# takkasila/practical_path_guiding_lab

Measured on AMD Instinct MI355X. Metric: Msamples/s guided, veach-ajar 1920x1080 max_depth 13, higher is better.
Workload: dtype f32; 1 GPU; veach-ajar 1920x1080, max_depth 13, 16 one-sample training passes (main.py:192, 218) per step in one batched launch (the whole film), guided iteration 6 (SD-tree trained by rendering iterations 0-5, 252 spp); full PathGuidingIntegrator.sample(): camera rays, NEE, BSDF/SD-tree MIS, record list, po...; spp_per_pass=16, passes_per_launch=16, steps_per_launch=1, kd_leaves=21429, quad_records=1675769, jump_bits=6, kd_grid_bits=6, bytes_jump_tables=1404370944, pixels_per_rank_min=2073600, pixels_per_rank_max=2073600

## Files before the change

practical_path_guiding_lab_amd/csrc/pg_probe.hip:

```cpp
#include <string>
#include <type_traits>
#include <vector>

#include "pg_render_dev.hpp"
#include "pg_render_stages.hpp"
#include "pg_scene_state.hpp"

using namespace pg;

namespace {

constexpr uint64_t kProbeMaxRays = 1ull << 20;
static_assert(kProbeMaxRays * (uint64_t)kOvfStack <= 0xffffffffull, "pg_scene_intersect: the overflow strips are indexed by 32 bits");

struct ProbeArgs {
	Shapes shapes;
	uint64_t n;
	const float *o, *d, *tmax;
	float *t, *uv;
	int32_t *prim;
	uint2 *ovf;
};

template <int kLevel, bool kAny, int kForm>
__global__ __launch_bounds__(kRBlock) void k_probe_intersect(ProbeArgs p)
{
	constexpr int kStack = kForm == 1 ? kShadeStack : kLdsStack;
	constexpr int kTop = kForm == 1 ? kShadeTopNodes : kBvhTopNodes;
	__shared__ uint2 s_stack[kStack][kRBlock];
	const uint64_t tid = (uint64_t)blockIdx.x * kRBlock + threadIdx.x;
	BvhStack stk = bvh_stack(&s_stack[0][threadIdx.x], p.ovf, (uint32_t)tid * (uint32_t)kOvfStack, kStack);
	if (kForm != 2) {
		__shared__ u32x4_t s_top[kTop * kBvhNodeQuads];
		RenderArgs a;
		a.shapes = p.shapes;
		stage_bvh_top<kTop>(s_top, a, stk);
	}
	if (tid >= p.n) return;
	const v3 o = ld3(p.o + 3 * tid), d = ld3(p.d + 3 * tid);
	float t, bu = 0.0f, bv = 0.0f;
	const int prim = intersect<kLevel, kAny, kForm == 1>(p.shapes, o, d, p.tmax[tid], t, stk, bu, bv);
	p.t[tid] = t;
	p.prim[tid] = prim;
	p.uv[2 * tid] = bu;
	p.uv[2 * tid + 1] = bv;
}

template <int kLevel, bool kAny>
auto intersect_form(int form) -> void (*)(ProbeArgs)
{
	if (form == 0) return k_probe_intersect<kLevel, kAny, 0>;
	if (form == 1) return k_probe_intersect<kLevel, kAny, 1>;
	return k_probe_intersect<kLevel, kAny, 2>;
}
// ... 314 lines not shown
```

practical_path_guiding_lab_amd/csrc/pg_render_dev.hpp:

```cpp
#pragma once

#include "pg_context.hpp"
#include "pg_descent.hpp"
#include "pg_kernels.hpp"
#include "pg_scene_layout.hpp"

#define PG_OUTLINE __forceinline__

namespace pg {

constexpr int kRBlock = 256;
static_assert(kRBlock == kStageThreads, "stage_kd_planes copies one plane per thread");
constexpr float kInvPiF = 0.31830988618379067154f;
constexpr float kRayEps = 1e-4f;
constexpr float kShadowEps = 1e-3f;

struct v3 {
	float x, y, z;
};
__device__ __forceinline__ v3 V(float x, float y, float z) { v3 r = {x, y, z}; return r; }
__device__ __forceinline__ v3 vadd(v3 a, v3 b) { return V(a.x + b.x, a.y + b.y, a.z + b.z); }
__device__ __forceinline__ v3 vsub(v3 a, v3 b) { return V(a.x - b.x, a.y - b.y, a.z - b.z); }
__device__ __forceinline__ v3 vmul(v3 a, v3 b) { return V(a.x * b.x, a.y * b.y, a.z * b.z); }
__device__ __forceinline__ v3 vscale(v3 a, float s) { return V(a.x * s, a.y * s, a.z * s); }
// ... 62 lines not shown
typedef __attribute__((address_space(3))) uint32_t LdsWord;
typedef __attribute__((address_space(3))) u32x4_t LdsQuad;
struct BvhStack {
	LdsWord *lds;
	uint2 *ovf;
	uint32_t ovf_first;
	const LdsQuad *top;
	uint32_t n_top;
	int n_lds;
	__device__ __forceinline__ void push(int sp, uint32_t ref, float t) const
	{
		if (sp < n_lds) {
			lds[sp * (2 * kRBlock)] = ref;
			lds[sp * (2 * kRBlock) + 1] = __float_as_uint(t);
		} else ovf[ovf_first + (uint32_t)(sp - n_lds)] = make_uint2(ref, __float_as_uint(t));
	}
	__device__ __forceinline__ uint2 at(int sp) const
	{
		const volatile LdsWord *w = lds + (sp < n_lds ? sp : n_lds - 1) * (2 * kRBlock);
		uint2 e = make_uint2(w[0], w[1]);
		if (sp >= n_lds) e = ovf[ovf_first + (uint32_t)(sp - n_lds)];
		return e;
	}
	__device__ __forceinline__ void push_ref(int sp, uint32_t ref) const
	{
		if (sp < n_lds) lds[sp * (2 * kRBlock)] = ref;
		else ovf[ovf_first + (uint32_t)(sp - n_lds)].x = ref;
	}
	__device__ __forceinline__ uint32_t ref_at(int sp) const
	{
		const volatile LdsWord *w = lds + (sp < n_lds ? sp : n_lds - 1) * (2 * kRBlock);
		uint32_t r = w[0];
		if (sp >= n_lds) r = ovf[ovf_first + (uint32_t)(sp - n_lds)].x;
		return r;
	}
};
__device__ __forceinline__ BvhStack bvh_stack(uint2 *lds_column, uint2 *ovf, uint32_t ovf_first, int n_lds = kLdsStack)
{
	BvhStack s;
	s.n_lds = n_lds;
	s.lds = (LdsWord *)lds_column;
	s.ovf = ovf;
	s.ovf_first = ovf_first;
	s.top = nullptr; s.n_top = 0;
	return s;
}

__device__ __forceinline__ v3 box_face_normal(const float *B, int face)
{
	const v3 n = ld3(B + BOX_NORMALS + 3 * (face >> 1));
	return (face & 1) ? V(-n.x, -n.y, -n.z) : n;
}

__device__ __forceinline__ bool bvh_box_hit(float lox, float loy, float loz, float hix, float hiy, float hiz, v3 o,
                                            v3 inv, bool negx, bool negy, bool negz, float bt, float &tmin_out)
{
	const float nx = ((negx ? hix : lox) - o.x) * inv.x, fx = ((negx ? lox : hix) - o.x) * inv.x;
	const float ny = ((negy ? hiy : loy) - o.y) * inv.y, fy = ((negy ? loy : hiy) - o.y) * inv.y;
	const float nz = ((negz ? hiz : loz) - o.z) * inv.z, fz = ((negz ? loz : hiz) - o.z) * inv.z;
	const float tmin = __builtin_fmaxf(__builtin_fmaxf(__builtin_fmaxf(nx, ny), nz), 0.0f);
	const float tmax = __builtin_fminf(__builtin_fminf(__builtin_fminf(fx, fy), fz), bt);
	tmin_out = tmin;
	return tmin <= tmax * 1.0000004f;
}

__device__ __forceinline__ bool bvh_box_hit_nf(float nxp, float nyp, float nzp, float fxp, float fyp, float fzp, v3 o, v3 inv,
                                               float bt, float &tmin_out)
// ... 93 lines not shown
	int best, sp, budget;
	uint32_t next;
};
__device__ __forceinline__ void bvh_rows(v3 d, int &nx, int &fx, int &ny, int &fy, int &nz, int &fz)
{
	const bool ngx = (__float_as_uint(d.x) >> 31) != 0u, ngy = (__float_as_uint(d.y) >> 31) != 0u, ngz = (__float_as_uint(d.z) >> 31) != 0u;
	constexpr int lo = BVH_BOXES * 4, hi = lo + BVH_HI_ROW * (int)kBvhRowBytes, row = (int)kBvhRowBytes;
	nx = ngx ? hi : lo; fx = ngx ? lo : hi;
	ny = ngy ? hi + row : lo + row; fy = ngy ? lo + row : hi + row;
	nz = ngz ? hi + 2 * row : lo + 2 * row; fz = ngz ? lo + 2 * row : hi + 2 * row;
}

__device__ __forceinline__ void bvh_begin(BvhWalk &w, const Shapes &sh, v3 o, v3 d, float bt, int best)
{
	w.o = o; w.d = d;
	w.inv = V(1.0f / d.x, 1.0f / d.y, 1.0f / d.z);
	bvh_rows(d, w.row_nx, w.row_fx, w.row_ny, w.row_fy, w.row_nz, w.row_fz);
	w.bt = bt; w.bu = 0.0f; w.bv = 0.0f;
	w.best = best; w.sp = 0;
	w.budget = 8 * sh.n_bvh_nodes + 8;
	w.next = 0;
}

template <bool kSlim = false, bool kAny = false>
__device__ __forceinline__ void bvh_node_step(BvhWalk &w, const Shapes &sh, const BvhStack &stk)
{
	const float kInf = __builtin_huge_valf();
	int row_nx = w.row_nx, row_fx = w.row_fx, row_ny = w.row_ny, row_fy = w.row_fy, row_nz = w.row_nz, row_fz = w.row_fz;
	if (kSlim) {
		v3 d = w.d;
		asm volatile("" : "+v"(d.x), "+v"(d.y), "+v"(d.z));
		bvh_rows(d, row_nx, row_fx, row_ny, row_fy, row_nz, row_fz);
	}
	const char *B = reinterpret_cast<const char *>(sh.bvh);
	const uint32_t nb = w.next * kBvhNodeBytes;
	uint4 nx4, ny4, nz4, fx4, fy4, fz4, rf;
	if (w.next < stk.n_top) {
		const LdsQuad *T = stk.top + w.next * (uint32_t)kBvhNodeQuads;
#define PG_Q(r) ({ const u32x4_t q_ = T[r]; make_uint4(q_.x, q_.y, q_.z, q_.w); })
		nx4 = PG_Q(row_nx >> 4); ny4 = PG_Q(row_ny >> 4); nz4 = PG_Q(row_nz >> 4);
		fx4 = PG_Q(row_fx >> 4); fy4 = PG_Q(row_fy >> 4); fz4 = PG_Q(row_fz >> 4); rf = PG_Q(BVH_REFS / BVH_WIDTH);
#undef PG_Q
	} else {
		nx4 = gather16(B + (nb + (uint32_t)row_nx)); ny4 = gather16(B + (nb + (uint32_t)row_ny)); nz4 = gather16(B + (nb + (uint32_t)row_nz));
		fx4 = gather16(B + (nb + (uint32_t)row_fx)); fy4 = gather16(B + (nb + (uint32_t)row_fy)); fz4 = gather16(B + (nb + (uint32_t)row_fz));
		rf = gather16(B + (nb + kBvhRefsByte));
	}
	uint32_t r0 = rf.x, r1 = rf.y, r2 = rf.z, r3 = rf.w;
	float t0, t1, t2, t3;
#define PG_F(v) __uint_as_float(v)
	const bool h0 = bvh_box_hit_nf(PG_F(nx4.x), PG_F(ny4.x), PG_F(nz4.x), PG_F(fx4.x), PG_F(fy4.x), PG_F(fz4.x), w.o, w.inv, w.bt, t0);
	const bool h1 = bvh_box_hit_nf(PG_F(nx4.y), PG_F(ny4.y), PG_F(nz4.y), PG_F(fx4.y), PG_F(fy4.y), PG_F(fz4.y), w.o, w.inv, w.bt, t1);
	const bool h2 = bvh_box_hit_nf(PG_F(nx4.z), PG_F(ny4.z), PG_F(nz4.z), PG_F(fx4.z), PG_F(fy4.z), PG_F(fz4.z), w.o, w.inv, w.bt, t2);
	const bool h3 = bvh_box_hit_nf(PG_F(nx4.w), PG_F(ny4.w), PG_F(nz4.w), PG_F(fx4.w), PG_F(fy4.w), PG_F(fz4.w), w.o, w.inv, w.bt, t3);
#undef PG_F
	if (!(r0 != kBvhNone && h0)) { r0 = kBvhNone; t0 = kInf; }
	if (!(r1 != kBvhNone && h1)) { r1 = kBvhNone; t1 = kInf; }
	if (!(r2 != kBvhNone && h2)) { r2 = kBvhNone; t2 = kInf; }
	if (!(r3 != kBvhNone && h3)) { r3 = kBvhNone; t3 = kInf; }
	if (kAny) {
		const bool n0 = r0 != kBvhNone, n1 = !n0 && r1 != kBvhNone, n2 = !n0 && !n1 && r2 != kBvhNone;
		w.next = n0 ? r0 : (n1 ? r1 : (n2 ? r2 : r3));
		if (n1) r1 = kBvhNone;
		if (n2) r2 = kBvhNone;
		if (!n0 && !n1 && !n2) r3 = kBvhNone;
		if (r3 != kBvhNone) { stk.push_ref(w.sp, r3); ++w.sp; }
		if (r2 != kBvhNone) { stk.push_ref(w.sp, r2); ++w.sp; }
		if (r1 != kBvhNone) { stk.push_ref(w.sp, r1); ++w.sp; }
		--w.budget;
		return;
	}
	bvh_cswap(t0, r0, t1, r1);
	bvh_cswap(t2, r2, t3, r3);
	bvh_cswap(t0, r0, t2, r2);
	bvh_cswap(t1, r1, t3, r3);
	bvh_cswap(t1, r1, t2, r2);
	if (r3 != kBvhNone) { stk.push(w.sp, r3, t3); ++w.sp; }
	if (r2 != kBvhNone) { stk.push(w.sp, r2, t2); ++w.sp; }
	if (r1 != kBvhNone) { stk.push(w.sp, r1, t1); ++w.sp; }
	w.next = r0;
	--w.budget;
}

__device__ __forceinline__ void bvh_tri_test(BvhWalk &w, v3 v0, v3 e1, v3 e2, int prim)
{
	const v3 o = w.o, d = w.d;
	const v3 p = V(d.y * e2.z - d.z * e2.y, d.z * e2.x - d.x * e2.z, d.x * e2.y - d.y * e2.x);
	const float det = dot3(e1, p);
	if (det == 0.0f) return;
	const float inv_det = 1.0f / det;
	const v3 s = vsub(o, v0);
	const float u = dot3(s, p) * inv_det;
	if (!(u >= 0.0f && u <= 1.0f)) return;
	const v3 q = V(s.y * e1.z - s.z * e1.y, s.z * e1.x - s.x * e1.z, s.x * e1.y - s.y * e1.x);
	const float v = dot3(d, q) * inv_det;
	if (!(v >= 0.0f && u + v <= 1.0f)) return;
	const float t = dot3(e2, q) * inv_det;
	if (t > 0.0f && t < w.bt) { w.bt = t; w.best = prim; w.bu = u; w.bv = v; }
}

__device__ __forceinline__ void bvh_leaf_step(BvhWalk &w, const Shapes &sh, int tri_base)
{
	const uint32_t first = bvh_leaf_first(w.next), count = bvh_leaf_count(w.next);
	for (uint32_t i = first; i < first + count; ++i) {
		const float *T = sh.tris + (size_t)i * kTriStride;
		v3 v0 = ld3(T + TRI_V0);
		const v3 e1 = ld3(T + TRI_E1), e2 = ld3(T + TRI_E2);
		asm volatile("" : "+v"(v0.x), "+v"(v0.y), "+v"(v0.z));
		bvh_tri_test(w, v0, e1, e2, tri_base + (int)i);
	}
}

template <bool kAny = false>
__device__ __forceinline__ void bvh_pop(BvhWalk &w, const BvhStack &stk)
{
	w.next = kBvhNone;
	if (kAny) {
		if (w.sp && w.budget > 0) {
			--w.sp;
			w.next = stk.ref_at(w.sp);
			--w.budget;
		}
		return;
	}
	while (w.sp && w.next == kBvhNone && w.budget > 0) {
		--w.sp;
		const uint2 e = stk.at(w.sp);
		if (__uint_as_float(e.y) <= w.bt * 1.0000004f) w.next = e.x;
		--w.budget;
	}
}

template <int kGeneral, bool kAny = false, bool kSlim = false>
__device__ __forceinline__ int intersect(const Shapes &sh, v3 o, v3 d, float tmax, float &t_out, const BvhStack &stk,
                                         float &bu, float &bv)
{
	int best = -1;
	float bt = tmax;
	intersect_linear<kGeneral>(sh, o, d, bt, best);
	if (kGeneral >= 2 && sh.n_bvh_nodes && !(kAny && best >= 0)) {
		const int tri_base = sh.first_tri();
		BvhWalk w;
		bvh_begin(w, sh, o, d, bt, best);
		while (true) {
			while (!(w.next & kBvhLeafBit) && w.budget > 0) {
				bvh_node_step<kSlim, kAny>(w, sh, stk);
				if (w.next == kBvhNone) bvh_pop<kAny>(w, stk);
			}
			if (w.next != kBvhNone && (w.next & kBvhLeafBit)) {
				bvh_leaf_step(w, sh, tri_base);
				if (kAny && w.best >= 0) break;
			}
			bvh_pop<kAny>(w, stk);
			if (w.next == kBvhNone) break;
		}
		bt = w.bt; best = w.best;
		if (w.best >= tri_base) { bu = w.bu; bv = w.bv; }
	}
	t_out = bt;
	return best;
}


template <int kGeneral, bool kAny = false>
__device__ __forceinline__ int intersect(const Shapes &sh, v3 o, v3 d, float tmax, float &t_out)
{
	static_assert(kGeneral < 2, "mesh scenes pass their BVH stack");
	const BvhStack none = bvh_stack(nullptr, nullptr, 0u);
	float bu, bv;
	return intersect<kGeneral, kAny>(sh, o, d, tmax, t_out, none, bu, bv);
}

__device__ __forceinline__ v3 texture_eval(const Shapes &sh, int index, float u, float v)
{
	const uint32_t *T = sh.textures + (size_t)index * kTextureStride;
	static_assert(TEX_KIND == 0 && TEX_WIDTH == 1 && TEX_HEIGHT == 2 && TEX_FIRST == 3 && TEX_COLOR0 == 4 && TEX_COLOR1 == 7 &&
	              TEX_UV_SCALE == 10 && TEX_UV_OFFSET == 12, "texture_eval names the words of the groups by .x .y .z .w");
	const uint4 t0 = *reinterpret_cast<const uint4 *>(T + TEX_KIND), t2 = *reinterpret_cast<const uint4 *>(T + TEX_COLOR1 + 1),
	            t3 = *reinterpret_cast<const uint4 *>(T + TEX_UV_OFFSET);
	const float uu = __uint_as_float(t2.z) * u + __uint_as_float(t3.x);
	const float vv = __uint_as_float(t2.w) * v + __uint_as_float(t3.y);
	if (t0.x == TEX_CHECKERBOARD) {
		const uint4 t1 = *reinterpret_cast<const uint4 *>(T + TEX_COLOR0);
		const float fu = uu - __builtin_floorf(uu), fv = vv - __builtin_floorf(vv);
		const bool mx = fu > 0.5f, my = fv > 0.5f;
		return mx == my ? V(__uint_as_float(t1.x), __uint_as_float(t1.y), __uint_as_float(t1.z))
		                : V(__uint_as_float(t1.w), __uint_as_float(t2.x), __uint_as_float(t2.y));
	}
	const int W = (int)t0.y, H = (int)t0.z;
	float x = uu * (float)W - 0.5f, y = vv * (float)H - 0.5f;
	if (!(fabs_(x) < 1e9f)) x = 0.0f;
	if (!(fabs_(y) < 1e9f)) y = 0.0f;
	const float fx = __builtin_floorf(x), fy = __builtin_floorf(y);
// ... 597 lines not shown
	uint32_t *prev_quad;
	uint8_t *hit0;
	uint64_t *rng_state, *rng_inc;
	uint32_t *ray_of;
	float *r_bsdf, *r_tb, *r_tr, *r_nee, *r_wp;
	uint2 *r_slot;
	uint32_t *r_tree;
	const uint4 *st_in;
	uint4 *st_out;
	const uint64_t *inc_in;
	uint64_t *inc_out;
	uint16_t *sort_key;
	const uint32_t *perm;
	uint32_t n_sort;
	uint4 *carry_in, *carry_out;
	uint4 *Lq;
	uint32_t *ws;
	uint2 *bvh_ovf;
	uint32_t *cast_count, *shadow_count, *shadow_list;
};


constexpr int kBvhTopNodes = 48;
template <int kNodes>
__device__ __forceinline__ void stage_bvh_top(u32x4_t *s_top, const RenderArgs &a, BvhStack &stk)
{
	const uint32_t n = a.shapes.n_bvh_nodes < kNodes ? (uint32_t)a.shapes.n_bvh_nodes : (uint32_t)kNodes;
	constexpr int kLoads = (kNodes * kBvhNodeQuads + kRBlock - 1) / kRBlock;
	if (n) {
		u32x4_t v[kLoads];
#pragma unroll
		for (int k = 0; k < kLoads; ++k) {
			const uint32_t i = threadIdx.x + (uint32_t)k * kRBlock;
			v[k] = reinterpret_cast<const u32x4_t *>(a.shapes.bvh)[i < n * (uint32_t)kBvhNodeQuads ? i : 0u];
		}
#pragma unroll
		for (int k = 0; k < kLoads; ++k) {
			const uint32_t i = threadIdx.x + (uint32_t)k * kRBlock;
			if (i < n * (uint32_t)kBvhNodeQuads) s_top[i] = v[k];
		}
	}
	__syncthreads();
	stk.top = (const LdsQuad *)s_top;
	stk.n_top = n;
}
constexpr int kShadeTopNodes = 40;
constexpr int kShadeStack = 6;
static_assert(kShadeStack >= kMinLdsStack && kShadeStack <= kLdsStack, "k_wave_shade: LDS stack depth");

constexpr uint32_t kTailPaths = 128u * 1024u;
__host__ __device__ constexpr bool tail_checkpoint(int bounce, int max_depth)
{
	return max_depth > 8 && bounce >= 4 && bounce + 1 < max_depth &&
	       (bounce < 8 || (bounce < 16 && bounce % 2 == 0) || bounce % 4 == 0);
}
typedef const __attribute__((address_space(4))) uint32_t *ConstU32Ptr;
__device__ __forceinline__ uint32_t live_final(const RenderArgs &a, int j)
{
	return reinterpret_cast<ConstU32Ptr>(reinterpret_cast<uintptr_t>(a.live_count))[j];
}
__device__ __forceinline__ uint64_t records_before(const RenderArgs &a)
{
	uint64_t r = a.n_lanes;
	for (int j = 0; j + 1 < a.bounce; ++j) r += live_final(a, j);
	return r;
}

__device__ __forceinline__ bool tail_took_over(const RenderArgs &a, int bounce)
{
	if (a.max_depth <= 8) return false;
	for (int c = 4; c <= bounce; ++c)
// ... 56 lines not shown
```

practical_path_guiding_lab_amd/csrc/pg_render_wave.hip:

```cpp
#include "pg_render_stages.hpp"

namespace pg {

enum : int {
	WS_HIT_PRIM = 0, WS_HIT_T, WS_HIT_U, WS_HIT_V,
	WS_P, WS_NG = WS_P + 3,
	WS_FLAGS = WS_NG + 3,
	WS_U, WS_LE = WS_U + 10,
	WS_DS_D = WS_LE + 3, WS_DS_PDF = WS_DS_D + 3, WS_EM_W, WS_BV_EM = WS_EM_W + 3, WS_BP_EM = WS_BV_EM + 3,
	WS_SH_O, WS_SH_D = WS_SH_O + 3, WS_SH_T = WS_SH_D + 3,
	WS_WO_T, WS_ETA = WS_WO_T + 3,
	WS_RNG_LO, WS_RNG_HI,
	WS_OCC,
	WS_PDF_NEE, WS_PDF_TREE,
	WS_FWD, WS_FWD_THR = WS_FWD, WS_FWD_L = WS_FWD_THR + 4, WS_FWD_INC = WS_FWD_L + 4,
	WS_COUNT = WS_FWD_INC + 2
};

__device__ __forceinline__ void store_geo_position(const RenderArgs &a, uint32_t *geo, uint64_t rec_slot, v3 p)
{
	const uint64_t S = a.n_lanes * (uint64_t)a.max_depth;
	float *gf = reinterpret_cast<float *>(geo);
	PG_ST(gf + (GEO_P + 0) * S + rec_slot, p.x); PG_ST(gf + (GEO_P + 1) * S + rec_slot, p.y); PG_ST(gf + (GEO_P + 2) * S + rec_slot, p.z);
}
// ... 107 lines not shown
		ray_d = st_v3(q1);
		if (want_cls && tid < (uint64_t)a.n_sort)
			cls_ahead = (int)lane_class_ahead(st_u64(q0.w, q1.w), st_u64(q5.x, q5.y), a.frac);
	}
	HitRec h;
	h.u = 0.0f; h.v = 0.0f;
	h.prim = intersect<kLevel, false>(a.shapes, ray_o, ray_d, __builtin_huge_valf(), h.t, stk, h.u, h.v);
	if (a.carry_in) {
		*st_rec(a.carry_in, tid, PS_HIT) = st_q_hit(h);
		if (tid < (uint64_t)a.n_sort) a.sort_key[tid] = (uint16_t)(h.prim >= 0 ? vertex_sort_key(a, vadd(ray_o, vscale(ray_d, h.t)), cls_ahead) : 0xfffeu);
		return;
	}
	wsputu(a, WS_HIT_PRIM, tid, (uint32_t)h.prim);
	wsput(a, WS_HIT_T, tid, h.t);
	wsput(a, WS_HIT_U, tid, h.u);
	wsput(a, WS_HIT_V, tid, h.v);
}

constexpr int kRefillIdle = 16;
constexpr uint32_t kCastChunk = 128;
template <int kLevel, bool kFirst>
__global__ __launch_bounds__(kRBlock) __attribute__((amdgpu_waves_per_eu(7))) void k_wave_cast(RenderArgs a)
{
	__shared__ uint2 s_stack[kLdsStack][kRBlock];
	if (!kFirst && tail_took_over(a, a.bounce)) return;
	const uint32_t total = kFirst ? (uint32_t)a.n_lanes : live_final(a, a.bounce - 1);
	const uint32_t gtid = blockIdx.x * kRBlock + threadIdx.x, n_static = gridDim.x * kRBlock;
	if (blockIdx.x * kRBlock >= total) return;
	const unsigned wl = threadIdx.x & 63u;
	const Shapes &sh = a.shapes;
	__shared__ u32x4_t s_top[kBvhTopNodes * kBvhNodeQuads];
	BvhStack stk = bvh_stack(&s_stack[0][threadIdx.x], a.bvh_ovf, gtid * (uint32_t)kOvfStack);
	stage_bvh_top<kBvhTopNodes>(s_top, a, stk);
	const int tri_base = sh.first_tri();
	BvhWalk w;
	w.next = kBvhNone; w.sp = 0; w.budget = 0; w.best = -1; w.bt = 0.0f; w.bu = 0.0f; w.bv = 0.0f;
	bool has = false, first_round = true;
	bool exhausted = n_static >= total;
	uint32_t pool_next = 0, pool_end = 0;
	const uint32_t n_waves = n_static / 64u;
	uint64_t chunk = gtid / 64u;
	uint32_t my = 0;
	for (;;) {
		const unsigned long long idle = __ballot(!has);
		const uint32_t n_idle = (uint32_t)__popcll(idle);
		if (first_round || (!exhausted && n_idle >= (uint32_t)kRefillIdle)) {
			uint32_t idx = 0xffffffffu;
			if (first_round) idx = gtid;
			else {
				if (pool_next == pool_end) {
					const uint64_t begin = (uint64_t)n_static + chunk * kCastChunk;
					chunk += n_waves;
					if (begin >= (uint64_t)total) exhausted = true;
					else {
						pool_next = (uint32_t)begin;
// ... 281 lines not shown
			if (a.perm) {
				q2 = ws4(a, WS_FWD_THR, tid);
				q4 = ws4(a, WS_FWD_L, tid);
			} else {
				q2 = st_load(a.st_in, a, PS_THR, tid);
				q4 = st_load(a.st_in, a, PS_L, tid);
			}
			thr = st_v3(q2);
			ior = st_ior(q2);
			L = st_v3(q4);
			lane = st_lane(q4);
		}
		cont = stage_b<kLevel>(a, rng, thr, L, ior, A, g, occluded, lane, rec_base + tid, (uint32_t)a.bounce, ray_o, ray_d,
		                       prev_pdf, delta);
		p_here = A.p;
		if (kFirst) a.hit0[lane] = (A.flags & F_VALID) ? 1 : 0;
		if (!cont) end_path(a, lane, L);
	}
	append_survivors<kRBlock>(a, cont, ray_o, ray_d, thr, ior, delta, p_here, prev_pdf, L, lane, rng, s_wave, s_base, s_oct, s_rec);
}

constexpr int kShadeStage = 128;
constexpr int kShadeStash = 12;
constexpr int kShadeWalkQuads = kShadeStack * kRBlock / 2 + kShadeTopNodes * kBvhNodeQuads + kShadeStash * kRBlock / 4;
constexpr int kShadeLdsQuads = kShadeStage * PS_ENTRIES > kShadeWalkQuads ? kShadeStage * PS_ENTRIES : kShadeWalkQuads;
static_assert(PS_SPARE * kRBlock <= kShadeLdsQuads, "k_wave_shade: the records' seven entries per thread must fit the dynamic LDS");
template <int kLevel, bool kFirst>
__device__ __forceinline__ void shade_body(const RenderArgs &a)
{
	__shared__ float s_planes[3 * kKdGridPlanes];
	__shared__ uint32_t s_wave[kRBlock / 64];
	__shared__ uint32_t s_base;
	__shared__ uint32_t s_oct[kRBlock / 64][8];
	extern __shared__ uint4 s_dyn[];
	uint64_t tid;
	bool alive;
	if (!wave_entry<kFirst>(a, tid, alive)) return;
#ifndef PG_SHADE_PHASES
#define PG_SHADE_PHASES 0
#endif
#if PG_SHADE_PHASES
	__shared__ unsigned long long s_ph[kRBlock / 64][10];
	if ((threadIdx.x & 63u) == (unsigned)__builtin_ctzll(__ballot(1))) {
		s_ph[threadIdx.x >> 6][8] = (unsigned long long)clock64();
		s_ph[threadIdx.x >> 6][7] = 0ull;
	}
#define PG_PHASE(i)                                                                                                          \
	if (a.ph && (threadIdx.x & 63u) == (unsigned)__builtin_ctzll(__ballot(1))) {                                            \
		const unsigned long long t_now = (unsigned long long)clock64();                                                      \
		unsigned long long *row = s_ph[threadIdx.x >> 6];                                                                    \
		row[i] = t_now - row[8];                                                                                             \
		row[8] = t_now;                                                                                                      \
		row[7] |= 1ull << (i);                                                                                               \
	}
#else
#define PG_PHASE(i)
#endif
	constexpr int kPlaneLoads = 1, kTopLoads = (kShadeTopNodes * kBvhNodeQuads + kRBlock - 1) / kRBlock;
	float pl_pre[kPlaneLoads];
	u32x4_t top_pre[kTopLoads];
#pragma unroll
	for (int k = 0; k < kPlaneLoads; ++k) pl_pre[k] = 0.0f;
#pragma unroll
	for (int k = 0; k < kTopLoads; ++k) top_pre[k] = u32x4_t{0u, 0u, 0u, 0u};
	const uint32_t n_top = a.shapes.n_bvh_nodes < kShadeTopNodes ? (uint32_t)a.shapes.n_bvh_nodes : (uint32_t)kShadeTopNodes;
#pragma unroll
	for (int k = 0; k < kPlaneLoads; ++k)
		if (a.tree.kd_grid != nullptr && threadIdx.x + k * kRBlock < 3u * kKdGridPlanes) pl_pre[k] = a.tree.kd_planes[threadIdx.x + k * kRBlock];
#pragma unroll
	for (int k = 0; k < kTopLoads; ++k)
		if (threadIdx.x + k * kRBlock < n_top * 8u) top_pre[k] = reinterpret_cast<const u32x4_t *>(a.shapes.bvh)[threadIdx.x + k * kRBlock];
	uint4 cq0 = make_uint4(0u, 0u, 0u, 0u), cq1 = cq0, cq2 = cq0, cq3 = cq0, cq4 = cq0, cq5 = cq0, cq6 = cq0;
	uint32_t coop_place = (uint32_t)tid;
	const bool coop = !kFirst && a.perm != nullptr;
	if (coop) {
		if (alive && tid < (uint64_t)a.n_sort) coop_place = a.perm[tid];
		if (!alive) coop_place = 0u;
		const uint32_t l = threadIdx.x & 63u, wbase = threadIdx.x & ~63u, q = l & 7u;
		uint4 g[8];
#pragma unroll
		for (uint32_t k = 0; k < 8u; ++k) {
			const uint32_t j = k * 8u + (l >> 3);
			const uint32_t pj = (uint32_t)__shfl((int)coop_place, (int)j, 64);
			g[k] = gather16(st_rec(a.carry_in, pj, (int)q));
		}
#pragma unroll
		for (uint32_t k = 0; k < 8u; ++k)
			if (q < (uint32_t)PS_SPARE) s_dyn[q * kRBlock + wbase + k * 8u + (l >> 3)] = g[k];
		__builtin_amdgcn_fence(__ATOMIC_RELEASE, "wavefront");
		__builtin_amdgcn_wave_barrier();
		__builtin_amdgcn_fence(__ATOMIC_ACQUIRE, "wavefront");
		cq0 = s_dyn[PS_RAY_O * kRBlock + threadIdx.x]; cq1 = s_dyn[PS_RAY_D * kRBlock + threadIdx.x]; cq2 = s_dyn[PS_THR * kRBlock + threadIdx.x];
		cq3 = s_dyn[PS_PREV * kRBlock + threadIdx.x]; cq4 = s_dyn[PS_L * kRBlock + threadIdx.x]; cq5 = s_dyn[PS_INC * kRBlock + threadIdx.x];
		cq6 = s_dyn[PS_HIT * kRBlock + threadIdx.x];
		__syncthreads();
	}
	uint2 *s_stack = reinterpret_cast<uint2 *>(s_dyn);
	u32x4_t *s_top = reinterpret_cast<u32x4_t *>(s_dyn) + kShadeStack * kRBlock / 2;
	BvhStack stk = bvh_stack(s_stack + threadIdx.x, a.bvh_ovf, (uint32_t)tid * (uint32_t)kOvfStack, kShadeStack);
#pragma unroll
	for (int k = 0; k < kPlaneLoads; ++k)
		if (a.tree.kd_grid != nullptr && threadIdx.x + k * kRBlock < 3u * kKdGridPlanes) s_planes[threadIdx.x + k * kRBlock] = pl_pre[k];
	if (a.tree.kd_grid != nullptr)
		for (uint32_t i = threadIdx.x + kPlaneLoads * kRBlock; i < 3u * kKdGridPlanes; i += kRBlock) s_planes[i] = a.tree.kd_planes[i];
#pragma unroll
	for (int k = 0; k < kTopLoads; ++k)
		if (threadIdx.x + k * kRBlock < n_top * 8u) s_top[threadIdx.x + k * kRBlock] = top_pre[k];
	__syncthreads();
	stk.top = (const LdsQuad *)s_top;
	stk.n_top = n_top;
	bool cont = false;
	v3 ray_o = V(0, 0, 0), ray_d = V(0, 0, 1), thr = V(1, 1, 1), L = V(0, 0, 0), p_here = V(0, 0, 0), prev_p = V(0, 0, 0);
	float ior = 1.0f, prev_pdf = 1.0f;
	bool delta = false, prev_delta = true;
	uint64_t lane = tid;
	Pcg32 rng;
	rng.state = 0; rng.inc = 1;
	uint64_t rec_base = 0;
	if (!kFirst) {
		rec_base = records_before(a);
		rec_base = (uint64_t)__builtin_amdgcn_readfirstlane((uint32_t)rec_base) |
		           ((uint64_t)__builtin_amdgcn_readfirstlane((uint32_t)(rec_base >> 32)) << 32);
	}
	if (alive) {
		HitRec h;
		const bool from_rec = !kFirst && a.perm != nullptr;
		uint32_t place = (uint32_t)tid;
		if (!coop && from_rec && tid < (uint64_t)a.n_sort) place = a.perm[tid];
		if (kFirst) {
			camera_ray(a, tid, rng, ray_o, ray_d);
			h.u = 0.0f; h.v = 0.0f;
			h.prim = intersect<kLevel, false, true>(a.shapes, ray_o, ray_d, __builtin_huge_valf(), h.t, stk, h.u, h.v);
		} else if (from_rec) {
// ... 9 lines not shown
			prev_delta = st_delta(q2);
			prev_p = st_v3(q3);
			prev_pdf = st_wf(q3);
			h = st_hit(q6);
		} else {
			const uint4 q0 = st_load(a.st_in, a, PS_RAY_O, tid), q1 = st_load(a.st_in, a, PS_RAY_D, tid);
			rng.state = st_u64(q0.w, q1.w);
			rng.inc = a.inc_in[tid];
			ray_o = st_v3(q0); ray_d = st_v3(q1);
			const uint4 q2 = st_load(a.st_in, a, PS_THR, tid), q3 = st_load(a.st_in, a, PS_PREV, tid);
			thr = st_v3(q2);
			{ const uint4 q4 = st_load(a.st_in, a, PS_L, tid); ior = st_ior(q2); L = st_v3(q4); lane = st_lane(q4); }
			prev_delta = st_delta(q2);
			prev_p = st_v3(q3);
			prev_pdf = st_wf(q3);
			h = ws_hit(a, tid);
		}
		StageA A;
		PG_PHASE(0)
		stage_a1<kLevel>(a, rng, ray_o, ray_d, thr, prev_p, prev_pdf, prev_delta, h, (uint32_t)a.bounce, A);
		asm volatile("" : "+v"(A.flags), "+v"(A.wi.x), "+v"(A.wi.y), "+v"(A.wi.z), "+v"(A.p.x), "+v"(A.p.y), "+v"(A.p.z),
		                  "+v"(A.ng.x), "+v"(A.ng.y), "+v"(A.ng.z), "+v"(A.refl.x), "+v"(A.refl.y), "+v"(A.refl.z));
		asm volatile("" : "+v"(A.ds_d.x), "+v"(A.ds_d.y), "+v"(A.ds_d.z), "+v"(A.ds_pdf), "+v"(A.bp_em), "+v"(A.n.x), "+v"(A.n.y), "+v"(A.n.z));
		float *stash = reinterpret_cast<float *>(s_dyn) + (kShadeStack * kRBlock * 2 + kShadeTopNodes * 32) + threadIdx.x;
		stash[0 * kRBlock] = A.Le.x; stash[1 * kRBlock] = A.Le.y; stash[2 * kRBlock] = A.Le.z;
		stash[3 * kRBlock] = A.bv_em.x; stash[4 * kRBlock] = A.bv_em.y; stash[5 * kRBlock] = A.bv_em.z;
		stash[6 * kRBlock] = A.em_w.x; stash[7 * kRBlock] = A.em_w.y; stash[8 * kRBlock] = A.em_w.z;
		stash[9 * kRBlock] = thr.x; stash[10 * kRBlock] = thr.y; stash[11 * kRBlock] = thr.z;
		bool occluded = false;
		PG_PHASE(1)
		if (a.dc) {
			const unsigned long long m = __ballot((A.flags & F_NEED_SHADOW) != 0u);
			if ((threadIdx.x & 63u) == (unsigned)__builtin_ctzll(__ballot(1))) {
				atomicAdd(&a.dc->body_waves, 1ull);
				if (m) { atomicAdd(&a.dc->shadow_waves, 1ull); atomicAdd(&a.dc->shadow_lanes, (unsigned long long)__popcll(m)); }
			}
		}
		if (A.flags & F_NEED_SHADOW) {
			float th, bu, bv;
			occluded = intersect<kLevel, true, true>(a.shapes, A.sh_o, A.sh_d, A.sh_tmax, th, stk, bu, bv) >= 0;
		}
		PG_PHASE(2)
		asm volatile("" : "+v"(A.n.x), "+v"(A.n.y), "+v"(A.n.z), "+v"(A.mat));
		stage_a2<kLevel>(a, rng, A);
		asm volatile("" : "+v"(A.wo.x), "+v"(A.wo.y), "+v"(A.wo.z), "+v"(A.bsdf_w.x), "+v"(A.bsdf_w.y), "+v"(A.bsdf_w.z),
		                  "+v"(A.bsdf_pdf), "+v"(A.flags));
		if (kLevel >= 3) asm volatile("" : "+v"(A.eta));
		GuideOut g = guide_none(A.wo);
		PG_PHASE(3)
		if (guide_has_work(a, A.flags)) stage_guide(a, s_planes, rng, A.p, A.ds_d, (A.flags & F_SMP_TREE) ? V(0, 0, 0) : A.wo, A.flags, g);
		if (a.record && (A.flags & F_VALID)) store_slots(a, rec_base + tid, g);
		PG_PHASE(4)
		asm volatile("" : "+v"(A.n.x), "+v"(A.n.y), "+v"(A.n.z), "+v"(A.mat));
		A.Le = V(stash[0 * kRBlock], stash[1 * kRBlock], stash[2 * kRBlock]);
		A.bv_em = V(stash[3 * kRBlock], stash[4 * kRBlock], stash[5 * kRBlock]);
		A.em_w = V(stash[6 * kRBlock], stash[7 * kRBlock], stash[8 * kRBlock]);
		thr = V(stash[9 * kRBlock], stash[10 * kRBlock], stash[11 * kRBlock]);
		cont = stage_b<kLevel>(a, rng, thr, L, ior, A, g, occluded, lane, rec_base + tid, (uint32_t)a.bounce, ray_o, ray_d, prev_pdf, delta);
		p_here = A.p;
		if (kFirst) a.hit0[lane] = (A.flags & F_VALID) ? 1 : 0;
		if (!cont) end_path(a, lane, L);
		PG_PHASE(5)
	}
// ... 57 lines not shown
		} else {
			q0 = st_load(a.st_in, a, PS_RAY_O, tid); q1 = st_load(a.st_in, a, PS_RAY_D, tid); q2 = st_load(a.st_in, a, PS_THR, tid);
			q3 = st_load(a.st_in, a, PS_PREV, tid); q4 = st_load(a.st_in, a, PS_L, tid);
			rng.inc = a.inc_in[tid];
		}
		rng.state = st_u64(q0.w, q1.w);
		ray_o = st_v3(q0); ray_d = st_v3(q1); thr = st_v3(q2); prev_p = st_v3(q3);
		ior = st_ior(q2);
		prev_delta = st_delta(q2);
		prev_pdf = st_wf(q3);
		L = st_v3(q4);
		lane = st_lane(q4);
	}
	for (int depth = a.bounce; depth < a.max_depth; ++depth) {
		if (alive) {
			HitRec h;
			h.u = 0.0f; h.v = 0.0f;
			h.prim = intersect<kLevel, false>(a.shapes, ray_o, ray_d, __builtin_huge_valf(), h.t, stk, h.u, h.v);
			StageA A;
			stage_a<kLevel>(a, rng, ray_o, ray_d, thr, prev_p, prev_pdf, prev_delta, h, (uint32_t)depth, A);
			bool occluded = false;
			if (A.flags & F_NEED_SHADOW) {
				float th, bu, bv;
				occluded = intersect<kLevel, true>(a.shapes, A.sh_o, A.sh_d, A.sh_tmax, th, stk, bu, bv) >= 0;
			}
			GuideOut g = guide_none(A.wo);
			if constexpr (kGeo) {
				if (a.record && (A.flags & F_VALID)) store_geo_position(a, geo.planes, slot, A.p);
			}
			if (guide_has_work(a, A.flags)) stage_guide(a, s_planes, rng, A.p, A.ds_d, A.wo, A.flags, g);
			if (a.record && (A.flags & F_VALID)) store_slots(a, slot, g);
			if constexpr (kGeo) {
				if (a.record && (A.flags & F_VALID)) store_geo_directions(a, geo.planes, slot, g, (uint32_t)depth);
			}
			bool delta;
			alive = stage_b<kLevel>(a, rng, thr, L, ior, A, g, occluded, lane, slot, (uint32_t)depth, ray_o, ray_d, prev_pdf, delta);
			prev_p = A.p;
			prev_delta = delta;
			if (!alive) end_path(a, lane, L);
		}
		if (!tail_next_slot(a, depth, alive, tail_base, slot)) break;
	}
}

template <class K>
static dim3 persistent_grid(K kernel, unsigned &cached_per_cu, unsigned n_cus, uint64_t n_rays)
{
// ... 62 lines not shown
```

Baseline: 762.1 Msamples/s.

## Give any-hit BVH walks a reference-only stack and more LDS top nodes

```diff
diff --git a/practical_path_guiding_lab_amd/csrc/pg_probe.hip b/practical_path_guiding_lab_amd/csrc/pg_probe.hip
--- a/practical_path_guiding_lab_amd/csrc/pg_probe.hip
+++ b/practical_path_guiding_lab_amd/csrc/pg_probe.hip
@@ -25,11 +25,14 @@
 template <int kLevel, bool kAny, int kForm>
 __global__ __launch_bounds__(kRBlock) void k_probe_intersect(ProbeArgs p)
 {
-	constexpr int kStack = kForm == 1 ? kShadeStack : kLdsStack;
-	constexpr int kTop = kForm == 1 ? kShadeTopNodes : kBvhTopNodes;
-	__shared__ uint2 s_stack[kStack][kRBlock];
-	const uint64_t tid = (uint64_t)blockIdx.x * kRBlock + threadIdx.x;
-	BvhStack stk = bvh_stack(&s_stack[0][threadIdx.x], p.ovf, (uint32_t)tid * (uint32_t)kOvfStack, kStack);
+	constexpr int kStack = kAny ? (kForm == 0 ? kCastRefs : kForm == 1 ? kShadeRefs : kMinLdsStack) : (kForm == 1 ? kShadeStack : kLdsStack);
+	constexpr int kTop = kForm == 1 ? (kAny ? kShadeAnyTopNodes : kShadeTopNodes) : kBvhTopNodes;
+	__shared__ uint32_t s_stack[kStack * (kAny ? 1 : 2)][kRBlock];
+	const uint64_t tid = (uint64_t)blockIdx.x * kRBlock + threadIdx.x;
+	using Stack = std::conditional_t<kAny, BvhRefStack, BvhStack>;
+	Stack stk;
+	if constexpr (kAny) stk = bvh_ref_stack(&s_stack[0][threadIdx.x], p.ovf, (uint32_t)tid * (uint32_t)kOvfStack, kStack);
+	else stk = bvh_stack(reinterpret_cast<uint2 *>(&s_stack[0][0]) + threadIdx.x, p.ovf, (uint32_t)tid * (uint32_t)kOvfStack, kStack);
 	if (kForm != 2) {
 		__shared__ u32x4_t s_top[kTop * kBvhNodeQuads];
 		RenderArgs a;
diff --git a/practical_path_guiding_lab_amd/csrc/pg_render_dev.hpp b/practical_path_guiding_lab_amd/csrc/pg_render_dev.hpp
--- a/practical_path_guiding_lab_amd/csrc/pg_render_dev.hpp
+++ b/practical_path_guiding_lab_amd/csrc/pg_render_dev.hpp
@@ -1,4 +1,6 @@
 #pragma once
+
+#include <type_traits>
 
 #include "pg_context.hpp"
 #include "pg_descent.hpp"
@@ -108,18 +110,6 @@
 		if (sp >= n_lds) e = ovf[ovf_first + (uint32_t)(sp - n_lds)];
 		return e;
 	}
-	__device__ __forceinline__ void push_ref(int sp, uint32_t ref) const
-	{
-		if (sp < n_lds) lds[sp * (2 * kRBlock)] = ref;
-		else ovf[ovf_first + (uint32_t)(sp - n_lds)].x = ref;
-	}
-	__device__ __forceinline__ uint32_t ref_at(int sp) const
-	{
-		const volatile LdsWord *w = lds + (sp < n_lds ? sp : n_lds - 1) * (2 * kRBlock);
-		uint32_t r = w[0];
-		if (sp >= n_lds) r = ovf[ovf_first + (uint32_t)(sp - n_lds)].x;
-		return r;
-	}
 };
 __device__ __forceinline__ BvhStack bvh_stack(uint2 *lds_column, uint2 *ovf, uint32_t ovf_first, int n_lds = kLdsStack)
 {
@@ -129,6 +119,46 @@
 	s.ovf = ovf;
 	s.ovf_first = ovf_first;
 	s.top = nullptr; s.n_top = 0;
+	return s;
+}
+struct BvhRefStack {
+	LdsWord *lds;
+	uint32_t *ovf;
+	uint32_t ovf_first;
+	const LdsQuad *top;
+	uint32_t n_top;
+	int n_lds, pitch;
+	__device__ __forceinline__ void push_ref(int sp, uint32_t ref) const
+	{
+		if (sp < n_lds) lds[sp * (pitch * kRBlock)] = ref;
+		else ovf[(size_t)(ovf_first + (uint32_t)(sp - n_lds)) * (size_t)pitch] = ref;
+	}
+	__device__ __forceinline__ uint32_t ref_at(int sp) const
+	{
+		const volatile LdsWord *w = lds + (sp < n_lds ? sp : n_lds - 1) * (pitch * kRBlock);
+		uint32_t r = w[0];
+		if (sp >= n_lds) r = ovf[(size_t)(ovf_first + (uint32_t)(sp - n_lds)) * (size_t)pitch];
+		return r;
+	}
+};
+__device__ __forceinline__ BvhRefStack bvh_ref_stack(uint32_t *lds_column, uint2 *ovf, uint32_t ovf_first, int n_lds)
+{
+	BvhRefStack s;
+	s.n_lds = n_lds; s.pitch = 1;
+	s.lds = (LdsWord *)lds_column;
+	s.ovf = reinterpret_cast<uint32_t *>(ovf);
+	s.ovf_first = ovf_first;
+	s.top = nullptr; s.n_top = 0;
+	return s;
+}
+__device__ __forceinline__ BvhRefStack bvh_ref_view(const BvhStack &k)
+{
+	BvhRefStack s;
+	s.n_lds = k.n_lds; s.pitch = 2;
+	s.lds = k.lds;
+	s.ovf = reinterpret_cast<uint32_t *>(k.ovf);
+	s.ovf_first = k.ovf_first;
+	s.top = k.top; s.n_top = k.n_top;
 	return s;
 }
 
@@ -268,9 +298,10 @@
 	w.next = 0;
 }
 
-template <bool kSlim = false, bool kAny = false>
-__device__ __forceinline__ void bvh_node_step(BvhWalk &w, const Shapes &sh, const BvhStack &stk)
-{
+template <bool kSlim = false, bool kAny = false, class Stack = BvhStack>
+__device__ __forceinline__ void bvh_node_step(BvhWalk &w, const Shapes &sh, const Stack &stk)
+{
+	static_assert(kAny == std::is_same<Stack, BvhRefStack>::value, "an any-hit walk keeps references alone, a closest-hit walk distances too");
 	const float kInf = __builtin_huge_valf();
 	int row_nx = w.row_nx, row_fx = w.row_fx, row_ny = w.row_ny, row_fy = w.row_fy, row_nz = w.row_nz, row_fz = w.row_fz;
 	if (kSlim) {
@@ -304,7 +335,7 @@
 	if (!(r1 != kBvhNone && h1)) { r1 = kBvhNone; t1 = kInf; }
 	if (!(r2 != kBvhNone && h2)) { r2 = kBvhNone; t2 = kInf; }
 	if (!(r3 != kBvhNone && h3)) { r3 = kBvhNone; t3 = kInf; }
-	if (kAny) {
+	if constexpr (kAny) {
 		const bool n0 = r0 != kBvhNone, n1 = !n0 && r1 != kBvhNone, n2 = !n0 && !n1 && r2 != kBvhNone;
 		w.next = n0 ? r0 : (n1 ? r1 : (n2 ? r2 : r3));
 		if (n1) r1 = kBvhNone;
@@ -314,18 +345,18 @@
 		if (r2 != kBvhNone) { stk.push_ref(w.sp, r2); ++w.sp; }
 		if (r1 != kBvhNone) { stk.push_ref(w.sp, r1); ++w.sp; }
 		--w.budget;
-		return;
-	}
-	bvh_cswap(t0, r0, t1, r1);
-	bvh_cswap(t2, r2, t3, r3);
-	bvh_cswap(t0, r0, t2, r2);
-	bvh_cswap(t1, r1, t3, r3);
-	bvh_cswap(t1, r1, t2, r2);
-	if (r3 != kBvhNone) { stk.push(w.sp, r3, t3); ++w.sp; }
-	if (r2 != kBvhNone) { stk.push(w.sp, r2, t2); ++w.sp; }
-	if (r1 != kBvhNone) { stk.push(w.sp, r1, t1); ++w.sp; }
-	w.next = r0;
-	--w.budget;
+	} else {
+		bvh_cswap(t0, r0, t1, r1);
+		bvh_cswap(t2, r2, t3, r3);
+		bvh_cswap(t0, r0, t2, r2);
+		bvh_cswap(t1, r1, t3, r3);
+		bvh_cswap(t1, r1, t2, r2);
+		if (r3 != kBvhNone) { stk.push(w.sp, r3, t3); ++w.sp; }
+		if (r2 != kBvhNone) { stk.push(w.sp, r2, t2); ++w.sp; }
+		if (r1 != kBvhNone) { stk.push(w.sp, r1, t1); ++w.sp; }
+		w.next = r0;
+		--w.budget;
+	}
 }
 
 __device__ __forceinline__ void bvh_tri_test(BvhWalk &w, v3 v0, v3 e1, v3 e2, int prim)
@@ -357,28 +388,29 @@
 	}
 }
 
-template <bool kAny = false>
-__device__ __forceinline__ void bvh_pop(BvhWalk &w, const BvhStack &stk)
-{
+template <bool kAny = false, class Stack = BvhStack>
+__device__ __forceinline__ void bvh_pop(BvhWalk &w, const Stack &stk)
+{
+	static_assert(kAny == std::is_same<Stack, BvhRefStack>::value, "see bvh_node_step");
 	w.next = kBvhNone;
-	if (kAny) {
+	if constexpr (kAny) {
 		if (w.sp && w.budget > 0) {
 			--w.sp;
 			w.next = stk.ref_at(w.sp);
 			--w.budget;
 		}
-		return;
-	}
-	while (w.sp && w.next == kBvhNone && w.budget > 0) {
-		--w.sp;
-		const uint2 e = stk.at(w.sp);
-		if (__uint_as_float(e.y) <= w.bt * 1.0000004f) w.next = e.x;
-		--w.budget;
-	}
-}
-
-template <int kGeneral, bool kAny = false, bool kSlim = false>
-__device__ __forceinline__ int intersect(const Shapes &sh, v3 o, v3 d, float tmax, float &t_out, const BvhStack &stk,
+	} else {
+		while (w.sp && w.next == kBvhNone && w.budget > 0) {
+			--w.sp;
+			const uint2 e = stk.at(w.sp);
+			if (__uint_as_float(e.y) <= w.bt * 1.0000004f) w.next = e.x;
+			--w.budget;
+		}
+	}
+}
+
+template <int kGeneral, bool kAny = false, bool kSlim = false, class Stack = BvhStack>
+__device__ __forceinline__ int intersect(const Shapes &sh, v3 o, v3 d, float tmax, float &t_out, const Stack &stk,
                                          float &bu, float &bv)
 {
 	int best = -1;
@@ -414,7 +446,8 @@
 	static_assert(kGeneral < 2, "mesh scenes pass their BVH stack");
 	const BvhStack none = bvh_stack(nullptr, nullptr, 0u);
 	float bu, bv;
-	return intersect<kGeneral, kAny>(sh, o, d, tmax, t_out, none, bu, bv);
+	if constexpr (kAny) return intersect<kGeneral, true>(sh, o, d, tmax, t_out, bvh_ref_view(none), bu, bv);
+	else return intersect<kGeneral, false>(sh, o, d, tmax, t_out, none, bu, bv);
 }
 
 __device__ __forceinline__ v3 texture_eval(const Shapes &sh, int index, float u, float v)
@@ -1058,8 +1091,8 @@
 
 
 constexpr int kBvhTopNodes = 48;
-template <int kNodes>
-__device__ __forceinline__ void stage_bvh_top(u32x4_t *s_top, const RenderArgs &a, BvhStack &stk)
+template <int kNodes, class Stack>
+__device__ __forceinline__ void stage_bvh_top(u32x4_t *s_top, const RenderArgs &a, Stack &stk)
 {
 	const uint32_t n = a.shapes.n_bvh_nodes < kNodes ? (uint32_t)a.shapes.n_bvh_nodes : (uint32_t)kNodes;
 	constexpr int kLoads = (kNodes * kBvhNodeQuads + kRBlock - 1) / kRBlock;
@@ -1083,6 +1116,12 @@
 constexpr int kShadeTopNodes = 40;
 constexpr int kShadeStack = 6;
 static_assert(kShadeStack >= kMinLdsStack && kShadeStack <= kLdsStack, "k_wave_shade: LDS stack depth");
+constexpr int kShadeRefs = 8;
+constexpr int kShadeAnyTopNodes = 72;
+static_assert(kShadeRefs >= kMinLdsStack, "k_wave_shade: LDS stack depth of the any-hit walks");
+static_assert(kShadeRefs * kRBlock * 4 + kShadeAnyTopNodes * (int)kBvhNodeBytes <= kShadeStack * kRBlock * 8 + kShadeTopNodes * (int)kBvhNodeBytes,
+              "k_wave_shade: the any-hit launches split the camera launch's bytes, no more");
+constexpr int kCastRefs = 2 * kLdsStack;
 
 constexpr uint32_t kTailPaths = 128u * 1024u;
 __host__ __device__ constexpr bool tail_checkpoint(int bounce, int max_depth)
diff --git a/practical_path_guiding_lab_amd/csrc/pg_render_wave.hip b/practical_path_guiding_lab_amd/csrc/pg_render_wave.hip
--- a/practical_path_guiding_lab_amd/csrc/pg_render_wave.hip
+++ b/practical_path_guiding_lab_amd/csrc/pg_render_wave.hip
@@ -153,7 +153,7 @@
 template <int kLevel, bool kFirst>
 __global__ __launch_bounds__(kRBlock) __attribute__((amdgpu_waves_per_eu(7))) void k_wave_cast(RenderArgs a)
 {
-	__shared__ uint2 s_stack[kLdsStack][kRBlock];
+	__shared__ uint32_t s_refs[kCastRefs][kRBlock];
 	if (!kFirst && tail_took_over(a, a.bounce)) return;
 	const uint32_t total = kFirst ? (uint32_t)a.n_lanes : live_final(a, a.bounce - 1);
 	const uint32_t gtid = blockIdx.x * kRBlock + threadIdx.x, n_static = gridDim.x * kRBlock;
@@ -161,7 +161,7 @@
 	const unsigned wl = threadIdx.x & 63u;
 	const Shapes &sh = a.shapes;
 	__shared__ u32x4_t s_top[kBvhTopNodes * kBvhNodeQuads];
-	BvhStack stk = bvh_stack(&s_stack[0][threadIdx.x], a.bvh_ovf, gtid * (uint32_t)kOvfStack);
+	BvhRefStack stk = bvh_ref_stack(&s_refs[0][threadIdx.x], a.bvh_ovf, gtid * (uint32_t)kOvfStack, kCastRefs);
 	stage_bvh_top<kBvhTopNodes>(s_top, a, stk);
 	const int tri_base = sh.first_tri();
 	BvhWalk w;
@@ -489,8 +489,14 @@
 
 constexpr int kShadeStage = 128;
 constexpr int kShadeStash = 12;
-constexpr int kShadeWalkQuads = kShadeStack * kRBlock / 2 + kShadeTopNodes * kBvhNodeQuads + kShadeStash * kRBlock / 4;
+template <bool kFirst> struct ShadeLds {
+	static constexpr int kTop = kFirst ? kShadeTopNodes : kShadeAnyTopNodes;
+	static constexpr int kStackWords = kFirst ? kShadeStack * kRBlock * 2 : kShadeRefs * kRBlock;
+	static constexpr int kWalkQuads = kStackWords / 4 + kTop * kBvhNodeQuads + kShadeStash * kRBlock / 4;
+};
+constexpr int kShadeWalkQuads = ShadeLds<true>::kWalkQuads > ShadeLds<false>::kWalkQuads ? ShadeLds<true>::kWalkQuads : ShadeLds<false>::kWalkQuads;
 constexpr int kShadeLdsQuads = kShadeStage * PS_ENTRIES > kShadeWalkQuads ? kShadeStage * PS_ENTRIES : kShadeWalkQuads;
+static_assert(kShadeLdsQuads * 16 <= 29696, "k_wave_shade: 29 696 B of dynamic LDS per workgroup -- what the kernel took when five workgroups per compute unit were measured");
 static_assert(PS_SPARE * kRBlock <= kShadeLdsQuads, "k_wave_shade: the records' seven entries per thread must fit the dynamic LDS");
 template <int kLevel, bool kFirst>
 __device__ __forceinline__ void shade_body(const RenderArgs &a)
@@ -523,14 +529,15 @@
 #else
 #define PG_PHASE(i)
 #endif
-	constexpr int kPlaneLoads = 1, kTopLoads = (kShadeTopNodes * kBvhNodeQuads + kRBlock - 1) / kRBlock;
+	constexpr int kTop = ShadeLds<kFirst>::kTop, kStackWords = ShadeLds<kFirst>::kStackWords;
+	constexpr int kPlaneLoads = 1, kTopLoads = (kTop * kBvhNodeQuads + kRBlock - 1) / kRBlock;
 	float pl_pre[kPlaneLoads];
 	u32x4_t top_pre[kTopLoads];
 #pragma unroll
 	for (int k = 0; k < kPlaneLoads; ++k) pl_pre[k] = 0.0f;
 #pragma unroll
 	for (int k = 0; k < kTopLoads; ++k) top_pre[k] = u32x4_t{0u, 0u, 0u, 0u};
-	const uint32_t n_top = a.shapes.n_bvh_nodes < kShadeTopNodes ? (uint32_t)a.shapes.n_bvh_nodes : (uint32_t)kShadeTopNodes;
+	const uint32_t n_top = a.shapes.n_bvh_nodes < kTop ? (uint32_t)a.shapes.n_bvh_nodes : (uint32_t)kTop;
 #pragma unroll
 	for (int k = 0; k < kPlaneLoads; ++k)
 		if (a.tree.kd_grid != nullptr && threadIdx.x + k * kRBlock < 3u * kKdGridPlanes) pl_pre[k] = a.tree.kd_planes[threadIdx.x + k * kRBlock];
@@ -563,8 +570,10 @@
 		__syncthreads();
 	}
 	uint2 *s_stack = reinterpret_cast<uint2 *>(s_dyn);
-	u32x4_t *s_top = reinterpret_cast<u32x4_t *>(s_dyn) + kShadeStack * kRBlock / 2;
+	u32x4_t *s_top = reinterpret_cast<u32x4_t *>(s_dyn) + kStackWords / 4;
 	BvhStack stk = bvh_stack(s_stack + threadIdx.x, a.bvh_ovf, (uint32_t)tid * (uint32_t)kOvfStack, kShadeStack);
+	BvhRefStack rstk = kFirst ? bvh_ref_view(stk)
+	                          : bvh_ref_stack(reinterpret_cast<uint32_t *>(s_dyn) + threadIdx.x, a.bvh_ovf, (uint32_t)tid * (uint32_t)kOvfStack, kShadeRefs);
 #pragma unroll
 	for (int k = 0; k < kPlaneLoads; ++k)
 		if (a.tree.kd_grid != nullptr && threadIdx.x + k * kRBlock < 3u * kKdGridPlanes) s_planes[threadIdx.x + k * kRBlock] = pl_pre[k];
@@ -574,8 +583,8 @@
 	for (int k = 0; k < kTopLoads; ++k)
 		if (threadIdx.x + k * kRBlock < n_top * 8u) s_top[threadIdx.x + k * kRBlock] = top_pre[k];
 	__syncthreads();
-	stk.top = (const LdsQuad *)s_top;
-	stk.n_top = n_top;
+	stk.top = (const LdsQuad *)s_top; rstk.top = stk.top;
+	stk.n_top = n_top; rstk.n_top = n_top;
 	bool cont = false;
 	v3 ray_o = V(0, 0, 0), ray_d = V(0, 0, 1), thr = V(1, 1, 1), L = V(0, 0, 0), p_here = V(0, 0, 0), prev_p = V(0, 0, 0);
 	float ior = 1.0f, prev_pdf = 1.0f;
@@ -631,7 +640,7 @@
 		asm volatile("" : "+v"(A.flags), "+v"(A.wi.x), "+v"(A.wi.y), "+v"(A.wi.z), "+v"(A.p.x), "+v"(A.p.y), "+v"(A.p.z),
 		                  "+v"(A.ng.x), "+v"(A.ng.y), "+v"(A.ng.z), "+v"(A.refl.x), "+v"(A.refl.y), "+v"(A.refl.z));
 		asm volatile("" : "+v"(A.ds_d.x), "+v"(A.ds_d.y), "+v"(A.ds_d.z), "+v"(A.ds_pdf), "+v"(A.bp_em), "+v"(A.n.x), "+v"(A.n.y), "+v"(A.n.z));
-		float *stash = reinterpret_cast<float *>(s_dyn) + (kShadeStack * kRBlock * 2 + kShadeTopNodes * 32) + threadIdx.x;
+		float *stash = reinterpret_cast<float *>(s_dyn) + (kStackWords + kTop * 32) + threadIdx.x;
 		stash[0 * kRBlock] = A.Le.x; stash[1 * kRBlock] = A.Le.y; stash[2 * kRBlock] = A.Le.z;
 		stash[3 * kRBlock] = A.bv_em.x; stash[4 * kRBlock] = A.bv_em.y; stash[5 * kRBlock] = A.bv_em.z;
 		stash[6 * kRBlock] = A.em_w.x; stash[7 * kRBlock] = A.em_w.y; stash[8 * kRBlock] = A.em_w.z;
@@ -647,7 +656,7 @@
 		}
 		if (A.flags & F_NEED_SHADOW) {
 			float th, bu, bv;
-			occluded = intersect<kLevel, true, true>(a.shapes, A.sh_o, A.sh_d, A.sh_tmax, th, stk, bu, bv) >= 0;
+			occluded = intersect<kLevel, true, true>(a.shapes, A.sh_o, A.sh_d, A.sh_tmax, th, rstk, bu, bv) >= 0;
 		}
 		PG_PHASE(2)
 		asm volatile("" : "+v"(A.n.x), "+v"(A.n.y), "+v"(A.n.z), "+v"(A.mat));
@@ -751,7 +760,7 @@
 			bool occluded = false;
 			if (A.flags & F_NEED_SHADOW) {
 				float th, bu, bv;
-				occluded = intersect<kLevel, true>(a.shapes, A.sh_o, A.sh_d, A.sh_tmax, th, stk, bu, bv) >= 0;
+				occluded = intersect<kLevel, true>(a.shapes, A.sh_o, A.sh_d, A.sh_tmax, th, bvh_ref_view(stk), bu, bv) >= 0;
 			}
 			GuideOut g = guide_none(A.wo);
 			if constexpr (kGeo) {
```

After: 759.2 Msamples/s, median of 3. Within noise of the previous version (-0.4%).
